# google/deepconsensus

Measured on NVIDIA H100. Metric: zmw_windows_per_sec, higher is better.
Workload: dtype bf16

## Files before the change

deepconsensus_b200/csrc/common.h:

```cpp
#pragma once
#include <cuda_bf16.h>
#include <stdint.h>

namespace dcb {

constexpr int kTileM = 128;
constexpr int kD = 280;
constexpr int kDP = 288;
constexpr int kHeads = 2;
constexpr int kDH = 140;
constexpr int kDHP = 144;
constexpr int kQKVN = 3 * kHeads * kDHP;
constexpr int kQKVGroup = 144;
constexpr int kNC = 144;
constexpr int kVocab = 5;
constexpr int kFFChunk = 128;

constexpr int kXChunks = kDP / 4;
__host__ __device__ inline size_t act_image_elems(int k) { return (size_t)kTileM * k; }
__host__ __device__ inline size_t x_image_elems() { return (size_t)kTileM * kDP; }

struct EmbedCol {
  int16_t src_row;
  int16_t width;
// ... 50 lines not shown
  float scale = 1.f;
};

struct RowEpi {
  float* x;
  __nv_bfloat16* xb;
  const float* bias;
  const float* pe;
  const float* pe_img;
  const float* ln_g;
  const float* ln_b;
  int has_xold;
  int L;
};

struct HeadParams {
  const float* x;
  const float* ln_g;
  const float* ln_b;
  const float* wfc;
  const float* bfc;
  const float* gw8;
  const float* ab;
  uint8_t* bases;
  uint8_t* quals;
  float* probs;
  float* logits;
  int M;
  int L, Lw;
  int calib_enabled;
// ... 7 lines not shown
```

deepconsensus_b200/csrc/engine.cu:

```cuda
#include <cuda_bf16.h>
#include <cuda_runtime.h>
#include <math.h>
#include <stdarg.h>
#include <stdio.h>
#include <string.h>

#include <algorithm>
#include <cmath>
#include <functional>
#include <map>
#include <memory>
#include <string>
#include <vector>

#include "../../include/dcb200.h"
#include "../../include/dcb200_debug.h"
#include "kernels.h"

using namespace dcb;

namespace {

thread_local std::string g_create_error;

// ... 97 lines not shown
  float prof_ms[kProfKinds] = {};
  int prof_n[kProfKinds] = {};
  long long prof_ffn_tokens = 0;
  float last_ms = 0.f;
  int last_launches = 0;
  int last_chunk_tokens = 0;
  std::vector<EmbedTable> tables;
  std::vector<StrictEmbedRow> embed;
  int table_elems = 0;
  Weights w;
  DevBuf<__nv_bfloat16> d_embqkv;
  DevBuf<float> d_x;
  DevBuf<__nv_bfloat16> d_xb;
  DevBuf<__nv_bfloat16> d_att;
  DevBuf<__nv_bfloat16> d_hid;
  DevBuf<double> d_p10;
  DevBuf<float> d_dbg;
  DevBuf<__nv_bfloat16> d_dbg_op;
  struct Strict {
    DevBuf<float> emb, x, y, q, k, v, att, hid;
    int chunk_windows = 0;
  } strict;
  struct {
    DevBuf<uint8_t> bases, quals, seq, qual, names, fastq;
    DevBuf<int32_t> start, len, pos, name_off, outcome;
    DevBuf<int64_t> rec_off, win_off;
    DevBuf<double> avg_q;
  } st;
  struct { DevBuf<int16_t> bq; DevBuf<uint8_t> mask; DevBuf<double> avg; } sk;
  struct {
// ... 477 lines not shown
    const int tl = t / e->L * e->Lw + t % e->L;
    const int tile = tl / kTileM, r = tl % kTileM;
    for (int col = 0; col < ow; ++col)
      out[(size_t)t * ow + col] = img[(((size_t)tile * (iw / K) + col / K) * kTileM + r) * K + col % K];
  }
  return DCB_OK;
}

void bf16_forward_chunk(dcb_engine* e, LaunchRecorder& rec, const float* rows_chunk, const uint8_t* packed_chunk,
                        int bw, HeadParams hp, int* d_status) {
  const dcb_config& c = e->cfg;
  const Weights& W = e->w;
  const int L = e->L, Lw = e->Lw, M = bw * Lw;
  const int T = (M + kTileM - 1) / kTileM;
  const cudaStream_t st = rec.st;
  int stage = 0;
  auto snap = [&]() {
    if (e->debug) {
      const size_t ximg = x_image_elems(), cw = (size_t)e->chunk_tiles * kTileM;
      cudaMemcpyAsync(e->d_dbg + (size_t)stage * e->chunk_tiles * ximg, e->d_x, T * ximg * sizeof(float), cudaMemcpyDeviceToDevice, st);
      size_t cols = 0;
      for (const DbgImage& im : dbg_images(e)) {
        if (im.stage == stage)
          cudaMemcpyAsync(e->d_dbg_op + cols * cw, im.src->p, (size_t)T * kTileM * im.width * sizeof(__nv_bfloat16),
                          cudaMemcpyDeviceToDevice, st);
        cols += im.width;
      }
    }
    ++stage;
  };
  rec.run(kProfEmbed, 1, [&] {
    launch_embed(rows_chunk, packed_chunk, e->pl, e->R, L, Lw, M, T, e->echunks, W.cols, W.rowmeta, W.tables,
                 e->table_elems, e->d_embqkv, d_status, st);
  });
  rec.run(kProfRowGemm, 1, [&] {
    launch_gemm_row(e->d_embqkv, W.wc, e->Epad / 16, 2 * (e->Epad / 16), T, row_epi(e, false, nullptr, 0, 0, true), st);
  });
  snap();
  for (int n_ = 0; n_ < c.num_hidden_layers; ++n_) {
    const LayerDev& ld = W.layers[n_];
    if (Lw == kTileM) {
      rec.run(kProfAttention, 2, [&] {
        __nv_bfloat16* qkv = e->debug ? e->d_embqkv.p : nullptr;
        for (int half = 0; half < 2; ++half)
          launch_qkv_attention(half, e->d_xb, ld.wqkv, L, c.attn_win_size, T, qkv, e->d_att, st);
      });
    } else {
      rec.run(kProfQkv, 1, [&] { launch_gemm_qkv(e->d_xb, ld.wqkv, T, e->d_embqkv, st); });
      rec.run(kProfAttention, 1, [&] { launch_attention(e->d_embqkv, e->d_att, L, Lw, c.attn_win_size, bw, st); });
    }
    rec.run(kProfRowGemm, 1, [&] {
      launch_gemm_row(e->d_att, ld.wo, kDP / 16, 2 * (kDP / 16), T, row_epi(e, true, nullptr, n_, 1, false), st);
    });
    snap();
    rec.run(kProfFfn, 2, [&] {
      const RowEpi epi = row_epi(e, true, ld.b2, n_ + 1, 0, false);
      __nv_bfloat16* hid = e->debug ? e->d_hid.p : nullptr;
      for (int half = 0; half < 2; ++half) launch_ffn(half, e->d_xb, ld.w1, ld.b1, ld.w2, c.filter_size, T, hid, epi, st);
    });
    if (e->profile) e->prof_ffn_tokens += (long long)bw * L;
    snap();
  }
  hp.x = e->d_x; hp.M = M; hp.L = L; hp.Lw = Lw;
  rec.run(kProfHead, 1, [&] { launch_head(hp, T, st); });
  e->last_chunk_tokens = M;
}

}

extern "C" {

const char* dcb_version(void) { return "dcb200 0.1.0 (sm_90a)"; }

const char* dcb_last_error(const dcb_engine* e) { return e ? e->err.c_str() : g_create_error.c_str(); }

int dcb_create(const dcb_config* cfg, dcb_engine** out) {
  if (!cfg || !out) return fail(nullptr, DCB_ERR_INVALID, "null argument");
  if (cfg->struct_size != (int32_t)sizeof(dcb_config))
    return fail(nullptr, DCB_ERR_INVALID, "dcb_config size mismatch: got %d, built with %zu",
// ... 13 lines not shown
  int ndev = 0;
  if (cudaGetDeviceCount(&ndev) != cudaSuccess || ndev == 0)
    return fail(nullptr, DCB_ERR_CUDA, "no CUDA device available (the dcb200 engine has no CPU fallback)");
  if (cfg->device < 0 || cfg->device >= ndev) return fail(nullptr, DCB_ERR_INVALID, "bad device ordinal %d", cfg->device);
  cudaDeviceProp prop;
  if (cudaGetDeviceProperties(&prop, cfg->device) != cudaSuccess || prop.major != 9)
    return fail(nullptr, DCB_ERR_CUDA, "device %d is not an sm_90 GPU (compute capability %d.%d)", cfg->device,
                prop.major, prop.minor);

  std::unique_ptr<dcb_engine> eng(new dcb_engine());
  dcb_engine* e = eng.get();
  e->cfg = *cfg;
  e->num_sms = prop.multiProcessorCount;
  e->L = cfg->max_length;
  e->Lw = e->L;
  bool align = true;
#ifdef DCB_DEV_SWITCHES
  if (const char* env = getenv("DCB_ALIGN")) align = atoi(env) != 0;
#endif
  if (align && e->L <= kTileM) e->Lw = kTileM;
  e->R = 4 * cfg->max_passes + (cfg->use_ccs_bq ? 6 : 5);
  e->pl = make_packed_layout(cfg->max_passes, cfg->max_length, cfg->use_ccs_bq ? 1 : 0);
  {
    auto table = [&](const char* layer, int vocab, int width) {
      const int off = (e->table_elems + 7) / 8 * 8;
      e->tables.push_back(EmbedTable{layer, vocab, width, off});
      e->table_elems = off + vocab * width;
      return e->tables.back();
    };
    auto rows = [&](const EmbedTable& tb, int n, float clip, int shift) {
      for (int r = 0; r < n; ++r) {
        e->embed.push_back(StrictEmbedRow{clip, shift, tb.vocab, tb.width, e->E, tb.off});
        e->E += tb.width;
      }
    };
// ... 32 lines not shown
    CU(e, kernels_init());
    std::vector<double> p10(256);
    for (int q = 0; q < 256; ++q) p10[q] = pow(10.0, (double)q / -10.0);
    int rc = upload(e, e->d_p10, p10);
    const size_t T = e->chunk_tiles, mtok = (size_t)cfg->max_batch * e->L;
    for (auto& sl : e->slots) {
      if (!rc) rc = alloc(e, sl.d_rows, (size_t)cfg->max_batch * e->R * e->L);
      if (!rc) rc = alloc(e, sl.d_status, 1);
      if (!rc) rc = alloc(e, sl.d_bases, mtok);
      if (!rc) rc = alloc(e, sl.d_quals, mtok);
    }
    if (!rc) rc = alloc(e, e->d_embqkv, T * kTileM * (size_t)std::max(e->Epad, kQKVN));
    if (!rc) rc = alloc(e, e->d_x, T * x_image_elems());
    if (!rc) rc = alloc(e, e->d_xb, T * act_image_elems(kDP));
    if (!rc) rc = alloc(e, e->d_att, T * act_image_elems(kDP));
    return rc;
  }();
  if (rc) {
    g_create_error = e->err;
    return rc;
  }
  *out = eng.release();
  return DCB_OK;
}

void dcb_destroy(dcb_engine* e) {
  if (!e) return;
  cudaSetDevice(e->cfg.device);
  delete e;
}
// ... 194 lines not shown
  if (!sl.used) { e->last_ms = 0.f; e->last_launches = 0; return DCB_OK; }
  CU(e, cudaSetDevice(e->cfg.device));
  CU(e, cudaEventSynchronize(sl.done));
  CU(e, cudaGetLastError());
  CU(e, cudaEventElapsedTime(&e->last_ms, sl.ev0, sl.ev1));
  e->last_launches = sl.launches;
  const int status = *sl.h_status;
  for (size_t i = 0; i < sl.prof_used; ++i) {
    const ProfRegion& r = sl.prof[i];
    float ms = 0.f;
    CU(e, cudaEventElapsedTime(&ms, r.start, r.end));
    e->prof_ms[r.kind] += ms;
    ++e->prof_n[r.kind];
  }
  sl.prof_used = 0;
  if (status & 1) return fail(e, DCB_ERR_INPUT_RANGE, "embedding id out of range in the input rows (clamped)");
  return DCB_OK;
}

int dcb_forward(dcb_engine* e, const float* rows, int32_t batch, uint32_t flags, uint8_t* bases_out,
                uint8_t* quals_out, float* probs_out, float* logits_out) {
  int64_t ticket = -1;
  int rc = dcb_submit(e, rows, batch, flags, bases_out, quals_out, probs_out, logits_out, &ticket);
  if (rc) return rc;
  return dcb_wait(e, ticket);
}

int dcb_last_forward_ms(dcb_engine* e, float* ms) {
  if (!e || !ms) return DCB_ERR_INVALID;
  *ms = e->last_ms;
// ... 727 lines not shown
```

deepconsensus_b200/csrc/kernels.cu:

```cuda
#include "kernels.h"

#include <cuda_bf16.h>
#include <math.h>
#include <stdio.h>
#include <stdlib.h>

#include "head_finish.cuh"
#include "sm90.cuh"

namespace dcb {


__global__ void __launch_bounds__(256)
embed_rows_kernel(const float* __restrict__ rows, const uint8_t* __restrict__ packed, PackedLayout pl, int R, int L,
                  int Lw, int M, int echunks,
                  const EmbedCol* __restrict__ cols, const EmbedRow* __restrict__ rowmeta,
                  const __nv_bfloat16* __restrict__ tables, int table_elems,
                  __nv_bfloat16* __restrict__ emb, int* __restrict__ status) {
  extern __shared__ __align__(1024) uint8_t smem[];
  __nv_bfloat16* s_tab = reinterpret_cast<__nv_bfloat16*>(smem);
  const int tab_bytes = (table_elems * 2 + 15) & ~15;
  EmbedCol* s_cols = reinterpret_cast<EmbedCol*>(smem + tab_bytes);
  const int cols_bytes = (echunks * 8 * (int)sizeof(EmbedCol) + 15) & ~15;
  uint16_t* s_ids = reinterpret_cast<uint16_t*>(smem + tab_bytes + cols_bytes);
  const int tile = blockIdx.x;
  for (int i = threadIdx.x; i < table_elems; i += blockDim.x) s_tab[i] = tables[i];
  for (int i = threadIdx.x; i < echunks * 8; i += blockDim.x) s_cols[i] = cols[i];
  for (int idx = threadIdx.x; idx < R * kTileM; idx += blockDim.x) {
    const int rr = idx / kTileM, r = idx % kTileM;
    const int tok = tile * kTileM + r;
    int id = 0;
    if (tok < M) {
      const int b = tok / Lw, l = tok - b * Lw;
      const EmbedRow m = rowmeta[rr];
// ... 29 lines not shown
          const EmbedCol c = s_cols[kc * 8 + 2 * j + h];
          uint32_t bits = 0;
          if (c.src_row >= 0) {
            const int id = s_ids[c.src_row * kTileM + r];
            bits = __bfloat16_as_ushort(s_tab[c.table_off + id * c.width + c.col]);
          }
          pr |= bits << (16 * h);
        }
        packed[j] = pr;
      }
      val = make_uint4(packed[0], packed[1], packed[2], packed[3]);
    }
    uint4* dst = reinterpret_cast<uint4*>(emb + ((size_t)tile * echunks + kc) * kTileM * 8) + r;
    *dst = val;
  }
}

enum { EPI_QKV = 0, EPI_ROW = 1 };

template <int BN, int NCH, bool kAres>
struct GemmCfg {
  static constexpr int kNI = NCH * BN;
  static constexpr int kSK = 2;
  static constexpr int kABytesPerK = 2 * kTileM * 16;
  static constexpr int kBBytesPerK = 2 * kNI * 16;
  static constexpr int kStageBytes = kSK * ((kAres ? 0 : kABytesPerK) + kBBytesPerK);
  static constexpr int kStages = 8;
  static constexpr int kShortStages = 4;
  static constexpr int kLongK = 32;
  __host__ __device__ static constexpr int stages(int kstages) {
// ... 107 lines not shown
          v1 = col + 1 < kD ? (v1 - mean) * rstd * s_vec[kDP + col + 1] + s_vec[2 * kDP + col + 1] : 0.f;
        }
        *reinterpret_cast<uint32_t*>(xb + (j * BN + jj * 8) * kTileM) = pack_bf16x2(v0, v1);
      }
  }
#pragma unroll
  for (int j = 0; j < NCH; ++j)
#pragma unroll
    for (int i = 0; i < BN / 2; ++i) acc[j][i] = 0.f;
}

template <int BN, int NCH, int EPI, bool kAres>
__global__ void __launch_bounds__(384, 1)
gemm_kernel(const __nv_bfloat16* __restrict__ a_img, const __nv_bfloat16* __restrict__ b_img, int a_ksteps, int ksteps,
            int ntiles,
            int ngroups, __nv_bfloat16* __restrict__ out_img, int out_chunks, RowEpi epi) {
  using Cfg = GemmCfg<BN, NCH, kAres>;
  static_assert(EPI != EPI_ROW || (Cfg::kNI == kDP && !kAres), "row epilogue needs the full 288-wide row");
  extern __shared__ __align__(1024) uint8_t smem[];
  uint8_t* a_res = smem;
  const int kstages = ksteps / Cfg::kSK;
  const int nst = Cfg::stages(kstages);
  uint8_t* stage_base = smem + Cfg::kAresBytes;
  uint64_t* full = reinterpret_cast<uint64_t*>(stage_base + nst * Cfg::kStageBytes);
  uint64_t* empty = full + nst;
  uint64_t* a_full = empty + nst;
  uint64_t* a_empty = a_full + 1;
  uint64_t* turn = a_empty + 1;
  float* s_vec = reinterpret_cast<float*>(stage_base + nst * Cfg::kStageBytes + 256);

  const int warp = threadIdx.x >> 5;
  const int lane = threadIdx.x & 31;
  if constexpr (EPI == EPI_ROW) row_vectors_to_smem(s_vec, epi);
  if (threadIdx.x == 0) {
    for (int i = 0; i < nst; ++i) {
      mbar_init(&full[i], 1);
      mbar_init(&empty[i], 256);
    }
    mbar_init(a_full, 1);
    mbar_init(a_empty, 256);
    mbar_init(&turn[0], 128);
    mbar_init(&turn[1], 128);
    mbar_fence_init();
  }
  __syncthreads();

  const int nitems = kAres ? (ntiles + 1) / 2 : ntiles * ngroups;
  const int gper = kAres ? ngroups : 1;
  const size_t a_tile_bytes = (size_t)a_ksteps * Cfg::kABytesPerK;
  const size_t b_group_bytes = (size_t)ksteps * Cfg::kBBytesPerK;

  if (warp >= 8) {
    setmaxnreg_dec<40>();
    if (warp == 8 && lane == 0) {
      uint32_t slot = 0, phase = 0, it = 0;
      for (int item = blockIdx.x; item < nitems; item += gridDim.x, ++it) {
        const int tile = kAres ? 2 * item : item / ngroups;
        const uint8_t* a_src = reinterpret_cast<const uint8_t*>(a_img) + tile * a_tile_bytes;
        if constexpr (kAres) {
          const uint32_t a_bytes = (uint32_t)((tile + 1 < ntiles ? 2 : 1) * a_tile_bytes);
          mbar_wait(a_empty, (it & 1) ^ 1);
          mbar_arrive_expect_tx(a_full, a_bytes);
          bulk_g2s(a_res, a_src, a_bytes, a_full);
        }
        for (int gi = 0; gi < gper; ++gi) {
          const int grp = kAres ? gi : item % ngroups;
          const uint8_t* b_src = reinterpret_cast<const uint8_t*>(b_img) + grp * b_group_bytes;
          for (int s = 0; s < kstages; ++s) {
            constexpr int kh = Cfg::kSK;
            mbar_wait(&empty[slot], phase ^ 1);
            uint8_t* st = stage_base + slot * Cfg::kStageBytes;
            if constexpr (kAres) {
              mbar_arrive_expect_tx(&full[slot], kh * Cfg::kBBytesPerK);
// ... 96 lines not shown
            const int row = row0 + 64 * mh + 8 * h;
#pragma unroll
            for (int j = 0; j < NCH; ++j)
#pragma unroll
              for (int jj = 0; jj < BN / 8; ++jj) {
                const int col = grp * Cfg::kNI + j * BN + jj * 8 + 2 * q;
                *reinterpret_cast<uint32_t*>(obase + ((size_t)(col >> 3) * kTileM + row) * 8 + (col & 7)) =
                    pack_bf16x2(accm[mh][j][jj * 4 + 2 * h], accm[mh][j][jj * 4 + 2 * h + 1]);
              }
          }
        if constexpr (kAres) pass_turn();
      } else {
        row_epilogue<BN, NCH>(accm[0], tile, row0, q, s_vec, epi);
      }
    }
  }
}

struct FfnCfg {
  static constexpr int kUpK = kDP / 16;
  static constexpr int kDownK = kFFChunk / 16;
  static constexpr int kABytesPerK = 2 * kTileM * 16;
  static constexpr int kW1Bytes = 2 * kFFChunk * 16;
  static constexpr int kW2Bytes = 2 * kDP * 16;
  static constexpr int kStageBytes = kW2Bytes;
  static constexpr int kB1Off = 2 * kW1Bytes;
  static constexpr int kB1Bytes = kFFChunk * 4;
  static constexpr int kStages = 16;
  static constexpr int kATileBytes = kUpK * kABytesPerK;
  static constexpr int kBarBytes = 512;
  static constexpr int kVecBytes = 3 * kDP * 4;
  static constexpr int kSmemBytes = kATileBytes + kStages * kStageBytes + kBarBytes + kVecBytes;
  static constexpr int kThreads = 384;
  static_assert(kSmemBytes <= 232448, "over the sm_90 opt-in shared memory per block");
  static_assert((2 * kStages + 2) * 8 <= kBarBytes, "the mbarriers (full, empty, a_full, a_empty) fit");
  static_assert(kB1Off + kB1Bytes <= kStageBytes && kUpK % 2 == 0, "a stage holds two W1 k-steps and b1");
};

template <bool kHid>
__global__ void __launch_bounds__(384, 1)
ffn_gemm_kernel(const __nv_bfloat16* __restrict__ xb_img, const __nv_bfloat16* __restrict__ w1_img,
                const float* __restrict__ b1, const __nv_bfloat16* __restrict__ w2_img, int ff, int tile_begin,
                int tile_end, __nv_bfloat16* __restrict__ hid, RowEpi epi) {
  using Cfg = FfnCfg;
  extern __shared__ __align__(1024) uint8_t smem[];
  uint8_t* a_res = smem;
  uint8_t* stage_base = smem + Cfg::kATileBytes;
  uint64_t* full = reinterpret_cast<uint64_t*>(stage_base + Cfg::kStages * Cfg::kStageBytes);
  uint64_t* empty = full + Cfg::kStages;
  uint64_t* a_full = empty + Cfg::kStages;
  uint64_t* a_empty = a_full + 1;
  float* s_vec = reinterpret_cast<float*>(reinterpret_cast<uint8_t*>(full) + Cfg::kBarBytes);
  const int nch = ff / kFFChunk;

  const int warp = threadIdx.x >> 5;
  const int lane = threadIdx.x & 31;
  row_vectors_to_smem(s_vec, epi);
  if (threadIdx.x == 0) {
    for (int i = 0; i < Cfg::kStages; ++i) {
      mbar_init(&full[i], 1);
      mbar_init(&empty[i], 256);
    }
    mbar_init(a_full, 1);
    mbar_init(a_empty, 256);
    mbar_fence_init();
  }
  __syncthreads();

  if (warp >= 8) {
    setmaxnreg_dec<24>();
    if (warp == 8 && lane == 0) {
      uint32_t slot = 0, phase = 0, it = 0;
      auto stage = [&](const uint8_t* src, uint32_t bytes, const float* b1_src, uint32_t b1_bytes) {
        mbar_wait(&empty[slot], phase ^ 1);
        uint8_t* st = stage_base + slot * Cfg::kStageBytes;
        mbar_arrive_expect_tx(&full[slot], bytes + b1_bytes);
        bulk_g2s(st, src, bytes, &full[slot]);
        if (b1_bytes) bulk_g2s(st + Cfg::kB1Off, b1_src, b1_bytes, &full[slot]);
        if (++slot == Cfg::kStages) { slot = 0; phase ^= 1; }
      };
      for (int tile = tile_begin + blockIdx.x; tile < tile_end; tile += gridDim.x, ++it) {
        mbar_wait(a_empty, (it & 1) ^ 1);
        mbar_arrive_expect_tx(a_full, Cfg::kATileBytes);
        bulk_g2s(a_res, reinterpret_cast<const uint8_t*>(xb_img) + (size_t)tile * Cfg::kATileBytes, Cfg::kATileBytes,
                 a_full);
        for (int c = 0; c < nch; ++c) {
          const uint8_t* w1 = reinterpret_cast<const uint8_t*>(w1_img) + (size_t)c * Cfg::kUpK * Cfg::kW1Bytes;
          for (int s = 0; s < Cfg::kUpK / 2; ++s)
            stage(w1 + (size_t)s * 2 * Cfg::kW1Bytes, 2 * Cfg::kW1Bytes, b1 + c * kFFChunk,
                  s + 1 == Cfg::kUpK / 2 ? Cfg::kB1Bytes : 0);
          const uint8_t* w2 = reinterpret_cast<const uint8_t*>(w2_img) + (size_t)c * Cfg::kDownK * Cfg::kW2Bytes;
          for (int kk = 0; kk < Cfg::kDownK; ++kk) stage(w2 + (size_t)kk * Cfg::kW2Bytes, Cfg::kW2Bytes, nullptr, 0);
        }
      }
    }
    return;
// ... 73 lines not shown
        if (kk > 0) {
          wgmma_fence_regs(af[kk - 1]);
          mbar_arrive(&empty[prev]);
        }
        prev = slot;
        next_slot();
      }
      wgmma_wait<0>();
      wgmma_fence_regs(acc[0]);
      wgmma_fence_regs(acc[1]);
      wgmma_fence_regs(af[Cfg::kDownK - 1]);
      mbar_arrive(&empty[prev]);
    }

    row_epilogue<kNC, 2, false>(acc, tile, row0, q, s_vec, epi);
  }
}

constexpr int kAttStride = 144;
constexpr int kAttChunks = kDHP / 8;

__device__ __forceinline__ void mma_bf16_16816(float (&c)[4], const uint32_t (&a)[4], uint32_t b0,
                                               uint32_t b1) {
  asm volatile(
      "mma.sync.aligned.m16n8k16.row.col.f32.bf16.bf16.f32 {%0,%1,%2,%3}, {%4,%5,%6,%7}, {%8,%9}, "
      "{%0,%1,%2,%3};"
      : "+f"(c[0]), "+f"(c[1]), "+f"(c[2]), "+f"(c[3])
      : "r"(a[0]), "r"(a[1]), "r"(a[2]), "r"(a[3]), "r"(b0), "r"(b1));
}

__device__ __forceinline__ void ldmatrix_x2_trans(uint32_t& r0, uint32_t& r1, uint32_t addr) {
// ... 218 lines not shown
  static constexpr int kKVBytes = kTileM * kAttStride * 2;
  static constexpr int kBarBytes = 256;
  static constexpr int kSmemBytes = kATileBytes + 2 * kKVBytes + kStages * kStageBytes + kBarBytes;
  static constexpr int kThreads = 384;
  static_assert(kSmemBytes <= 232448, "over the sm_90 opt-in shared memory per block");
  static_assert((2 * kStages + 2) * 8 <= kBarBytes, "the mbarriers (full, empty, a_full, a_empty) fit");
  static_assert((2 * kAK) % kSK == 0, "every stage holds kSK k-steps of one group");
  static_assert(kQKVGroup == kDHP && kQKVN == 6 * kQKVGroup, "one n-group is one head's q, k or v");
};

__device__ __forceinline__ int qkv_att_group(int i) {
  const int h = i / 3, part = i % 3;
  return part == 0 ? 2 + h : part == 1 ? 4 + h : h;
}

__device__ __forceinline__ void consumer_bar_sync() { asm volatile("bar.sync 1, 256;" ::: "memory"); }

template <bool kQkv>
__global__ void __launch_bounds__(384, 1)
qkv_attention_kernel(const __nv_bfloat16* __restrict__ xb_img, const __nv_bfloat16* __restrict__ b_img, int L,
                     int win, int tile_begin, int tile_end, __nv_bfloat16* __restrict__ qkv_img,
                     __nv_bfloat16* __restrict__ att) {
  using Cfg = QkvAttCfg;
  extern __shared__ __align__(1024) uint8_t smem[];
  uint8_t* a_res = smem;
  __nv_bfloat16* sK = reinterpret_cast<__nv_bfloat16*>(smem + Cfg::kATileBytes);
  __nv_bfloat16* sV = reinterpret_cast<__nv_bfloat16*>(smem + Cfg::kATileBytes + Cfg::kKVBytes);
  uint8_t* stage_base = smem + Cfg::kATileBytes + 2 * Cfg::kKVBytes;
  uint64_t* full = reinterpret_cast<uint64_t*>(stage_base + Cfg::kStages * Cfg::kStageBytes);
  uint64_t* empty = full + Cfg::kStages;
  uint64_t* a_full = empty + Cfg::kStages;
  uint64_t* a_empty = a_full + 1;

  const int warp = threadIdx.x >> 5;
  const int lane = threadIdx.x & 31;
  if (threadIdx.x == 0) {
    for (int i = 0; i < Cfg::kStages; ++i) {
      mbar_init(&full[i], 1);
      mbar_init(&empty[i], 256);
    }
    mbar_init(a_full, 1);
    mbar_init(a_empty, 256);
    mbar_fence_init();
  }
  __syncthreads();

  if (warp >= 8) {
    setmaxnreg_dec<24>();
    if (warp == 8 && lane == 0) {
      uint32_t slot = 0, phase = 0, it = 0;
      for (int tile = tile_begin + blockIdx.x; tile < tile_end; tile += gridDim.x, ++it) {
        mbar_wait(a_empty, (it & 1) ^ 1);
        mbar_arrive_expect_tx(a_full, Cfg::kATileBytes);
        bulk_g2s(a_res, reinterpret_cast<const uint8_t*>(xb_img) + (size_t)tile * Cfg::kATileBytes, Cfg::kATileBytes,
                 a_full);
        for (int i = 0; i < 6; ++i) {
          const uint8_t* b_src = reinterpret_cast<const uint8_t*>(b_img) + (size_t)qkv_att_group(i) * Cfg::kGroupBytes;
          for (int s = 0; s < Cfg::kGroupStages; ++s) {
            mbar_wait(&empty[slot], phase ^ 1);
            mbar_arrive_expect_tx(&full[slot], Cfg::kStageBytes);
            bulk_g2s(stage_base + slot * Cfg::kStageBytes, b_src + (size_t)s * Cfg::kStageBytes, Cfg::kStageBytes,
                     &full[slot]);
            if (++slot == Cfg::kStages) { slot = 0; phase ^= 1; }
          }
        }
      }
// ... 74 lines not shown
        } else {
          const bool v0 = row0 < L, v1 = row0 + 8 < L;
#pragma unroll
          for (int ks = 0; ks < kDHP / 16; ++ks) {
            qa[ks][0] = v0 ? pack_bf16x2(acc[8 * ks + 0], acc[8 * ks + 1]) : 0u;
            qa[ks][1] = v1 ? pack_bf16x2(acc[8 * ks + 2], acc[8 * ks + 3]) : 0u;
            qa[ks][2] = v0 ? pack_bf16x2(acc[8 * ks + 4], acc[8 * ks + 5]) : 0u;
            qa[ks][3] = v1 ? pack_bf16x2(acc[8 * ks + 6], acc[8 * ks + 7]) : 0u;
          }
        }
      }
      consumer_bar_sync();
      const int i0 = warp * 16;
      if (i0 < L) attend_block(qa, sK, sV, i0, L, band, att, tile * kTileM, h);
    }
  }
}

__global__ void __launch_bounds__(128)
head_kernel(HeadParams p) {
  __shared__ __align__(16) float sGW[kD * 8];
  __shared__ float sA[kVocab], sBj[kVocab];
  for (int i = threadIdx.x; i < kD * 2; i += blockDim.x)
    reinterpret_cast<float4*>(sGW)[i] = __ldg(reinterpret_cast<const float4*>(p.gw8) + i);
  if (threadIdx.x < kVocab) { sA[threadIdx.x] = p.ab[threadIdx.x]; sBj[threadIdx.x] = p.ab[8 + threadIdx.x]; }
  __syncthreads();
  const int tile = blockIdx.x, r = threadIdx.x;
  const int tok = tile * kTileM + r;
  if (tok >= p.M) return;
  const int wdw = tok / p.Lw, pos = tok - wdw * p.Lw;
  if (pos >= p.L) return;
  const size_t oidx = (size_t)wdw * p.L + pos;
  const float4* xrow = reinterpret_cast<const float4*>(p.x + (size_t)tile * x_image_elems()) + r;
  float s1 = 0.f, s2 = 0.f;
  float t[kVocab];
#pragma unroll
  for (int j = 0; j < kVocab; ++j) t[j] = 0.f;
  const float shift = xrow[0].x;
  constexpr int kHB = 10;
  static_assert((kD / 4) % kHB == 0, "head batch");
#pragma unroll 1
  for (int c0 = 0; c0 < kD / 4; c0 += kHB) {
// ... 9 lines not shown
        s1 += ys[i];
        s2 = fmaf(ys[i], ys[i], s2);
        const float4 w0 = *reinterpret_cast<const float4*>(&sGW[col * 8]);
        const float w4 = sGW[col * 8 + 4];
        t[0] = fmaf(ys[i], w0.x, t[0]); t[1] = fmaf(ys[i], w0.y, t[1]); t[2] = fmaf(ys[i], w0.z, t[2]);
        t[3] = fmaf(ys[i], w0.w, t[3]); t[4] = fmaf(ys[i], w4, t[4]);
      }
    }
  }
  const float m1 = s1 * (1.f / kD);
  const float rstd = rsqrtf(fmaxf(s2 * (1.f / kD) - m1 * m1, 0.f) + 1e-6f);
  float lg[kVocab];
#pragma unroll
  for (int j = 0; j < kVocab; ++j) lg[j] = rstd * (t[j] - m1 * sA[j]) + sBj[j];
  head_finish(p, lg, oidx);
}

static int g_num_sms = 0;
static int num_sms() {
  if (!g_num_sms) {
    int dev = 0;
    cudaGetDevice(&dev);
    cudaDeviceGetAttribute(&g_num_sms, cudaDevAttrMultiProcessorCount, dev);
    if (g_num_sms <= 0) g_num_sms = 132;
  }
  return g_num_sms;
}


template <int BN, int NCH, int EPI, bool kAres>
// ... 8 lines not shown
  if ((e = gemm_init<kNC, 1, EPI_QKV, true>()) != cudaSuccess) return e;
  for (auto fn : {ffn_gemm_kernel<false>, ffn_gemm_kernel<true>})
    if ((e = cudaFuncSetAttribute(fn, cudaFuncAttributeMaxDynamicSharedMemorySize, FfnCfg::kSmemBytes)) != cudaSuccess)
      return e;
  for (auto fn : {qkv_attention_kernel<false>, qkv_attention_kernel<true>})
    if ((e = cudaFuncSetAttribute(fn, cudaFuncAttributeMaxDynamicSharedMemorySize, QkvAttCfg::kSmemBytes)) !=
        cudaSuccess)
      return e;
  e = cudaFuncSetAttribute(embed_rows_kernel, cudaFuncAttributeMaxDynamicSharedMemorySize, 160 * 1024);
  if (e != cudaSuccess) return e;
  e = cudaFuncSetAttribute(band_attention_kernel, cudaFuncAttributeMaxDynamicSharedMemorySize,
                           2 * 256 * kAttStride * 2);
  return e;
}

size_t embed_smem_bytes(int R, int echunks, int table_elems) {
  return (size_t)((table_elems * 2 + 15) & ~15) + ((echunks * 8 * sizeof(EmbedCol) + 15) & ~(size_t)15) +
         (size_t)R * kTileM * 2;
}

void launch_embed(const float* rows, const uint8_t* packed, const PackedLayout& pl, int R, int L, int Lw, int M, int ntiles, int echunks,
                  const EmbedCol* cols, const EmbedRow* rowmeta, const __nv_bfloat16* tables,
                  int table_elems, __nv_bfloat16* emb, int* status, cudaStream_t st) {
  embed_rows_kernel<<<ntiles, 256, embed_smem_bytes(R, echunks, table_elems), st>>>(
      rows, packed, pl, R, L, Lw, M, echunks, cols, rowmeta, tables, table_elems, emb, status);
}

void launch_gemm_row(const __nv_bfloat16* a_img, const __nv_bfloat16* b_img, int a_ksteps, int b_ksteps, int ntiles,
                     const RowEpi& epi, cudaStream_t st) {
  using Cfg = GemmCfg<kNC, 2, false>;
  const int grid = ntiles < num_sms() ? ntiles : num_sms();
  const int smem = Cfg::smem_bytes(Cfg::stages(b_ksteps / Cfg::kSK));
  gemm_kernel<kNC, 2, EPI_ROW, false><<<grid, Cfg::kThreads, smem, st>>>(a_img, b_img, a_ksteps, b_ksteps, ntiles, 1,
                                                                                    nullptr, 0, epi);
}

void launch_gemm_qkv(const __nv_bfloat16* a_img, const __nv_bfloat16* b_img, int ntiles,
                     __nv_bfloat16* qkv_img, cudaStream_t st) {
  using Cfg = GemmCfg<kNC, 1, true>;
  const int npairs = (ntiles + 1) / 2;
  const int grid = npairs < num_sms() ? npairs : num_sms();
  RowEpi none{};
  gemm_kernel<kNC, 1, EPI_QKV, true><<<grid, Cfg::kThreads, Cfg::kSmemBytes, st>>>(
      a_img, b_img, kDP / 16, 2 * (kDP / 16), ntiles, kQKVN / kQKVGroup, qkv_img, kQKVN / 8, none);
}

void launch_ffn(int half, const __nv_bfloat16* xb_img, const __nv_bfloat16* w1_img, const float* b1,
                const __nv_bfloat16* w2_img, int ff, int ntiles, __nv_bfloat16* hid_img, const RowEpi& epi,
                cudaStream_t st) {
  const int split = (ntiles + 1) / 2;
  const int t0 = half ? split : 0, t1 = half ? ntiles : split;
  const int n = t1 - t0;
  const int grid = n < 1 ? 1 : n < num_sms() ? n : num_sms();
  if (hid_img)
    ffn_gemm_kernel<true><<<grid, FfnCfg::kThreads, FfnCfg::kSmemBytes, st>>>(xb_img, w1_img, b1, w2_img, ff, t0, t1,
                                                                              hid_img, epi);
  else
    ffn_gemm_kernel<false><<<grid, FfnCfg::kThreads, FfnCfg::kSmemBytes, st>>>(xb_img, w1_img, b1, w2_img, ff, t0, t1,
                                                                               nullptr, epi);
}

__global__ void __launch_bounds__(256)
unpack_rows_kernel(const uint8_t* __restrict__ packed, PackedLayout pl, int nwindows, float* __restrict__ rows) {
  const int b = blockIdx.x;
  const uint8_t* w = packed + (size_t)b * pl.stride;
  float* out = rows + (size_t)b * pl.R * pl.L;
  for (int i = threadIdx.x; i < pl.R * pl.L; i += blockDim.x) {
    const int r = i / pl.L, l = i - r * pl.L;
    out[i] = packed_value(pl, w, r, l);
  }
}

void launch_unpack_rows(const uint8_t* packed, const PackedLayout& pl, int nwindows, float* rows, cudaStream_t st) {
  if (nwindows > 0) unpack_rows_kernel<<<nwindows, 256, 0, st>>>(packed, pl, nwindows, rows);
}


void launch_attention(const __nv_bfloat16* qkv, __nv_bfloat16* att, int L, int Lw, int win, int nwindows,
                      cudaStream_t st) {
  const int Lp = (L + 15) & ~15;
  const size_t smem = (size_t)2 * Lp * kAttStride * 2;
  band_attention_kernel<<<nwindows * 2, 128, smem, st>>>(qkv, att, L, Lw, win, nwindows);
}

void launch_qkv_attention(int half, const __nv_bfloat16* xb_img, const __nv_bfloat16* wqkv, int L, int win,
                          int ntiles, __nv_bfloat16* qkv_img, __nv_bfloat16* att, cudaStream_t st) {
  const int split = (ntiles + 1) / 2;
  const int t0 = half ? split : 0, t1 = half ? ntiles : split;
  const int n = t1 - t0;
  const int grid = n < 1 ? 1 : n < num_sms() ? n : num_sms();
  if (qkv_img)
    qkv_attention_kernel<true><<<grid, QkvAttCfg::kThreads, QkvAttCfg::kSmemBytes, st>>>(xb_img, wqkv, L, win, t0, t1,
                                                                                        qkv_img, att);
  else
    qkv_attention_kernel<false><<<grid, QkvAttCfg::kThreads, QkvAttCfg::kSmemBytes, st>>>(xb_img, wqkv, L, win, t0,
                                                                                         t1, nullptr, att);
}



__global__ void __launch_bounds__(256)
stitch_kernel(const uint8_t* __restrict__ bases, const uint8_t* __restrict__ quals, int L,
              const int64_t* __restrict__ win_off, const int32_t* __restrict__ zmw_start, uint8_t* __restrict__ seq_out,
              uint8_t* __restrict__ qual_out, int32_t* __restrict__ len_out) {
  __shared__ int s_warp[8];
  __shared__ int s_total;
  const int z = blockIdx.x;
  const size_t off = (size_t)window_offset(win_off, zmw_start[z], L);
  const int n = (int)(window_offset(win_off, zmw_start[z + 1], L) - (int64_t)off);
  const uint8_t* in_b = bases + off;
  const uint8_t* in_q = quals + off;
// ... 33 lines not shown
        out_q[pos] = q[k];
        ++pos;
      }
    }
    running += s_total;
    __syncthreads();
  }
  if (threadIdx.x == 0) len_out[z] = running;
}

void launch_stitch(const uint8_t* bases, const uint8_t* quals, int L, const int64_t* win_off, const int32_t* zmw_start,
                   int n_zmw, uint8_t* seq_out, uint8_t* qual_out, int32_t* len_out, cudaStream_t st) {
  if (n_zmw > 0) stitch_kernel<<<n_zmw, 256, 0, st>>>(bases, quals, L, win_off, zmw_start, seq_out, qual_out, len_out);
}

void launch_head(const HeadParams& p, int ntiles, cudaStream_t st) {
  head_kernel<<<ntiles, 128, 0, st>>>(p);
}

}
```

deepconsensus_b200/csrc/kernels.h:

```cpp
#pragma once
#include <cuda_runtime.h>

#include "common.h"

namespace dcb {

cudaError_t kernels_init();

size_t embed_smem_bytes(int R, int echunks, int table_elems);
void launch_embed(const float* rows, const uint8_t* packed, const PackedLayout& pl, int R, int L, int Lw, int M, int ntiles, int echunks,
                  const EmbedCol* cols, const EmbedRow* rowmeta, const __nv_bfloat16* tables,
                  int table_elems, __nv_bfloat16* emb, int* status, cudaStream_t st);
void launch_gemm_row(const __nv_bfloat16* a_img, const __nv_bfloat16* b_img, int a_ksteps, int b_ksteps, int ntiles,
                     const RowEpi& epi, cudaStream_t st);
void launch_gemm_qkv(const __nv_bfloat16* a_img, const __nv_bfloat16* b_img, int ntiles,
                     __nv_bfloat16* qkv_img, cudaStream_t st);
void launch_ffn(int half, const __nv_bfloat16* xb_img, const __nv_bfloat16* w1_img, const float* b1,
                const __nv_bfloat16* w2_img, int ff, int ntiles, __nv_bfloat16* hid_img, const RowEpi& epi,
                cudaStream_t st);
void launch_unpack_rows(const uint8_t* packed, const PackedLayout& pl, int nwindows, float* rows, cudaStream_t st);
void launch_attention(const __nv_bfloat16* qkv, __nv_bfloat16* att, int L, int Lw, int win, int nwindows,
                      cudaStream_t st);
void launch_qkv_attention(int half, const __nv_bfloat16* xb_img, const __nv_bfloat16* wqkv, int L, int win,
                          int ntiles, __nv_bfloat16* qkv_img, __nv_bfloat16* att, cudaStream_t st);
void launch_head(const HeadParams& p, int ntiles, cudaStream_t st);
__host__ __device__ inline int64_t window_offset(const int64_t* win_off, int w, int L) {
  return win_off ? win_off[w] : (int64_t)w * L;
}
void launch_stitch(const uint8_t* bases, const uint8_t* quals, int L, const int64_t* win_off, const int32_t* zmw_start,
                   int n_zmw, uint8_t* seq_out, uint8_t* qual_out, int32_t* len_out, cudaStream_t st);


void launch_read_outcome(const uint8_t* qual, const int32_t* len, const int64_t* win_off, const int32_t* zmw_start,
                         const int32_t* window_pos, int L, int n_zmw, const double* p10, double min_quality, int min_length,
                         int32_t* outcome, double* avg_q, cudaStream_t st);
void launch_fastq(const uint8_t* seq, const uint8_t* qual, const int32_t* len, const int64_t* win_off, const int32_t* zmw_start,
                  int L, int n_zmw, const int32_t* outcome, const uint8_t* names, const int32_t* name_off, int64_t* rec_off,
                  uint8_t* fastq, int64_t cap, cudaStream_t st);
void launch_skip_mask(const int16_t* ccs_bq, int n_windows, int L, const double* p10, double thr, uint8_t* mask,
                      double* avg_out, cudaStream_t st);
// ... 72 lines not shown
```

Before: 165,000.

## Overlap forward kernels with PDL and per-tile release/acquire flags

Kernels in the forward pass are launched with programmatic stream serialization, so each can start while the one before is still running. Per-tile stamp flags in global memory, written with release stores and polled with acquire loads, let a consumer tile begin as soon as the matching producer tile is done, instead of waiting at a full kernel boundary. This targets launch gaps and tail idle time between the many kernels per layer. It adds spin-wait polling with a one-second timeout that reports an error, plus stamp bookkeeping, and it risks deadlock or extra contention if CTAs of the dependent kernel take SM slots the producer still needs.

```diff
diff --git a/deepconsensus_b200/csrc/common.h b/deepconsensus_b200/csrc/common.h
--- a/deepconsensus_b200/csrc/common.h
+++ b/deepconsensus_b200/csrc/common.h
@@ -88,6 +88,13 @@
   int L;
 };
 
+struct TileFlow {
+  int* flags;
+  int wait, done;
+  int* status;
+};
+constexpr int kStatusTileWait = 2;
+
 struct HeadParams {
   const float* x;
   const float* ln_g;
diff --git a/deepconsensus_b200/csrc/engine.cu b/deepconsensus_b200/csrc/engine.cu
--- a/deepconsensus_b200/csrc/engine.cu
+++ b/deepconsensus_b200/csrc/engine.cu
@@ -135,6 +135,9 @@
   DevBuf<__nv_bfloat16> d_xb;
   DevBuf<__nv_bfloat16> d_att;
   DevBuf<__nv_bfloat16> d_hid;
+  DevBuf<int> d_flow;
+  uint32_t flow_stamp = 0;
+  bool tile_flow = false;
   DevBuf<double> d_p10;
   DevBuf<float> d_dbg;
   DevBuf<__nv_bfloat16> d_dbg_op;
@@ -642,6 +645,23 @@
   const int L = e->L, Lw = e->Lw, M = bw * Lw;
   const int T = (M + kTileM - 1) / kTileM;
   const cudaStream_t st = rec.st;
+  const bool flow = e->tile_flow;
+  const uint32_t nstamps = 3 + 3 * (uint32_t)c.num_hidden_layers;
+  if (flow && e->flow_stamp > UINT32_MAX - nstamps) {
+    cudaMemsetAsync(e->d_flow, 0, e->chunk_tiles * sizeof(int), st);
+    e->flow_stamp = 0;
+  }
+  auto next_flow = [&](bool advance = true) {
+    TileFlow f{};
+    if (flow) {
+      f.flags = e->d_flow;
+      f.status = d_status;
+      f.wait = (int)e->flow_stamp;
+      f.done = (int)(e->flow_stamp + 1);
+      if (advance) ++e->flow_stamp;
+    }
+    return f;
+  };
   int stage = 0;
   auto snap = [&]() {
     if (e->debug) {
@@ -659,10 +679,11 @@
   };
   rec.run(kProfEmbed, 1, [&] {
     launch_embed(rows_chunk, packed_chunk, e->pl, e->R, L, Lw, M, T, e->echunks, W.cols, W.rowmeta, W.tables,
-                 e->table_elems, e->d_embqkv, d_status, st);
+                 e->table_elems, e->d_embqkv, d_status, next_flow(), st);
   });
   rec.run(kProfRowGemm, 1, [&] {
-    launch_gemm_row(e->d_embqkv, W.wc, e->Epad / 16, 2 * (e->Epad / 16), T, row_epi(e, false, nullptr, 0, 0, true), st);
+    launch_gemm_row(e->d_embqkv, W.wc, e->Epad / 16, 2 * (e->Epad / 16), T, row_epi(e, false, nullptr, 0, 0, true),
+                    next_flow(), st);
   });
   snap();
   for (int n_ = 0; n_ < c.num_hidden_layers; ++n_) {
@@ -671,26 +692,28 @@
       rec.run(kProfAttention, 2, [&] {
         __nv_bfloat16* qkv = e->debug ? e->d_embqkv.p : nullptr;
         for (int half = 0; half < 2; ++half)
-          launch_qkv_attention(half, e->d_xb, ld.wqkv, L, c.attn_win_size, T, qkv, e->d_att, st);
+          launch_qkv_attention(half, e->d_xb, ld.wqkv, L, c.attn_win_size, T, qkv, e->d_att, next_flow(half == 1), st);
       });
     } else {
       rec.run(kProfQkv, 1, [&] { launch_gemm_qkv(e->d_xb, ld.wqkv, T, e->d_embqkv, st); });
       rec.run(kProfAttention, 1, [&] { launch_attention(e->d_embqkv, e->d_att, L, Lw, c.attn_win_size, bw, st); });
     }
     rec.run(kProfRowGemm, 1, [&] {
-      launch_gemm_row(e->d_att, ld.wo, kDP / 16, 2 * (kDP / 16), T, row_epi(e, true, nullptr, n_, 1, false), st);
+      launch_gemm_row(e->d_att, ld.wo, kDP / 16, 2 * (kDP / 16), T, row_epi(e, true, nullptr, n_, 1, false), next_flow(),
+                      st);
     });
     snap();
     rec.run(kProfFfn, 2, [&] {
       const RowEpi epi = row_epi(e, true, ld.b2, n_ + 1, 0, false);
       __nv_bfloat16* hid = e->debug ? e->d_hid.p : nullptr;
-      for (int half = 0; half < 2; ++half) launch_ffn(half, e->d_xb, ld.w1, ld.b1, ld.w2, c.filter_size, T, hid, epi, st);
+      for (int half = 0; half < 2; ++half)
+        launch_ffn(half, e->d_xb, ld.w1, ld.b1, ld.w2, c.filter_size, T, hid, epi, next_flow(half == 1), st);
     });
     if (e->profile) e->prof_ffn_tokens += (long long)bw * L;
     snap();
   }
   hp.x = e->d_x; hp.M = M; hp.L = L; hp.Lw = Lw;
-  rec.run(kProfHead, 1, [&] { launch_head(hp, T, st); });
+  rec.run(kProfHead, 1, [&] { launch_head(hp, T, next_flow(), st); });
   e->last_chunk_tokens = M;
 }
 
@@ -734,11 +757,13 @@
   e->num_sms = prop.multiProcessorCount;
   e->L = cfg->max_length;
   e->Lw = e->L;
-  bool align = true;
+  bool align = true, tile_flow = true;
 #ifdef DCB_DEV_SWITCHES
   if (const char* env = getenv("DCB_ALIGN")) align = atoi(env) != 0;
+  if (const char* env = getenv("DCB_TILE_FLOW")) tile_flow = atoi(env) != 0;
 #endif
   if (align && e->L <= kTileM) e->Lw = kTileM;
+  e->tile_flow = tile_flow && e->Lw == kTileM;
   e->R = 4 * cfg->max_passes + (cfg->use_ccs_bq ? 6 : 5);
   e->pl = make_packed_layout(cfg->max_passes, cfg->max_length, cfg->use_ccs_bq ? 1 : 0);
   {
@@ -801,6 +826,7 @@
     if (!rc) rc = alloc(e, e->d_x, T * x_image_elems());
     if (!rc) rc = alloc(e, e->d_xb, T * act_image_elems(kDP));
     if (!rc) rc = alloc(e, e->d_att, T * act_image_elems(kDP));
+    if (!rc && e->tile_flow) rc = alloc(e, e->d_flow, T);
     return rc;
   }();
   if (rc) {
@@ -1025,6 +1051,9 @@
     ++e->prof_n[r.kind];
   }
   sl.prof_used = 0;
+  if (status & kStatusTileWait)
+    return fail(e, DCB_ERR_CUDA, "a launch of the forward waited over a second for a tile of the launch before it; "
+                                 "the outputs are not valid");
   if (status & 1) return fail(e, DCB_ERR_INPUT_RANGE, "embedding id out of range in the input rows (clamped)");
   return DCB_OK;
 }
diff --git a/deepconsensus_b200/csrc/kernels.cu b/deepconsensus_b200/csrc/kernels.cu
--- a/deepconsensus_b200/csrc/kernels.cu
+++ b/deepconsensus_b200/csrc/kernels.cu
@@ -10,14 +10,43 @@
 
 namespace dcb {
 
+__device__ __forceinline__ void pdl_launch_dependents() { asm volatile("griddepcontrol.launch_dependents;" ::: "memory"); }
+__device__ __forceinline__ void pdl_wait() { asm volatile("griddepcontrol.wait;" ::: "memory"); }
+
+__device__ __forceinline__ int ld_acquire_gpu(const int* p) {
+  int v;
+  asm volatile("ld.acquire.gpu.global.b32 %0, [%1];" : "=r"(v) : "l"(p) : "memory");
+  return v;
+}
+
+__device__ __forceinline__ void tile_wait(const TileFlow& f, int tile) {
+  if (!f.flags) return;
+  if (ld_acquire_gpu(f.flags + tile) == f.wait) return;
+  uint64_t t0, t;
+  asm volatile("mov.u64 %0, %%globaltimer;" : "=l"(t0));
+  while (ld_acquire_gpu(f.flags + tile) != f.wait) {
+    __nanosleep(100);
+    asm volatile("mov.u64 %0, %%globaltimer;" : "=l"(t));
+    if (t - t0 > 1000000000ull) { atomicOr(f.status, kStatusTileWait); return; }
+  }
+}
+
+__device__ __forceinline__ void fence_proxy_async() { asm volatile("fence.proxy.async.global;" ::: "memory"); }
+
+__device__ __forceinline__ void tile_done(const TileFlow& f, int tile) {
+  if (f.flags) asm volatile("st.release.gpu.global.b32 [%0], %1;" ::"l"(f.flags + tile), "r"(f.done) : "memory");
+}
+
+__device__ __forceinline__ void consumer_bar_sync() { asm volatile("bar.sync 1, 256;" ::: "memory"); }
 
 __global__ void __launch_bounds__(256)
 embed_rows_kernel(const float* __restrict__ rows, const uint8_t* __restrict__ packed, PackedLayout pl, int R, int L,
                   int Lw, int M, int echunks,
                   const EmbedCol* __restrict__ cols, const EmbedRow* __restrict__ rowmeta,
                   const __nv_bfloat16* __restrict__ tables, int table_elems,
-                  __nv_bfloat16* __restrict__ emb, int* __restrict__ status) {
+                  __nv_bfloat16* __restrict__ emb, int* __restrict__ status, TileFlow flow) {
   extern __shared__ __align__(1024) uint8_t smem[];
+  pdl_launch_dependents();
   __nv_bfloat16* s_tab = reinterpret_cast<__nv_bfloat16*>(smem);
   const int tab_bytes = (table_elems * 2 + 15) & ~15;
   EmbedCol* s_cols = reinterpret_cast<EmbedCol*>(smem + tab_bytes);
@@ -77,6 +106,8 @@
     uint4* dst = reinterpret_cast<uint4*>(emb + ((size_t)tile * echunks + kc) * kTileM * 8) + r;
     *dst = val;
   }
+  __syncthreads();
+  if (threadIdx.x == 0) tile_done(flow, tile);
 }
 
 enum { EPI_QKV = 0, EPI_ROW = 1 };
@@ -214,7 +245,7 @@
 __global__ void __launch_bounds__(384, 1)
 gemm_kernel(const __nv_bfloat16* __restrict__ a_img, const __nv_bfloat16* __restrict__ b_img, int a_ksteps, int ksteps,
             int ntiles,
-            int ngroups, __nv_bfloat16* __restrict__ out_img, int out_chunks, RowEpi epi) {
+            int ngroups, __nv_bfloat16* __restrict__ out_img, int out_chunks, RowEpi epi, TileFlow flow) {
   using Cfg = GemmCfg<BN, NCH, kAres>;
   static_assert(EPI != EPI_ROW || (Cfg::kNI == kDP && !kAres), "row epilogue needs the full 288-wide row");
   extern __shared__ __align__(1024) uint8_t smem[];
@@ -244,6 +275,7 @@
     mbar_fence_init();
   }
   __syncthreads();
+  pdl_launch_dependents();
 
   const int nitems = kAres ? (ntiles + 1) / 2 : ntiles * ngroups;
   const int gper = kAres ? ngroups : 1;
@@ -257,6 +289,8 @@
       for (int item = blockIdx.x; item < nitems; item += gridDim.x, ++it) {
         const int tile = kAres ? 2 * item : item / ngroups;
         const uint8_t* a_src = reinterpret_cast<const uint8_t*>(a_img) + tile * a_tile_bytes;
+        tile_wait(flow, tile);
+        fence_proxy_async();
         if constexpr (kAres) {
           const uint32_t a_bytes = (uint32_t)((tile + 1 < ntiles ? 2 : 1) * a_tile_bytes);
           mbar_wait(a_empty, (it & 1) ^ 1);
@@ -383,7 +417,12 @@
         row_epilogue<BN, NCH>(accm[0], tile, row0, q, s_vec, epi);
       }
     }
-  }
+    if (flow.flags) {
+      consumer_bar_sync();
+      if (threadIdx.x == 0) tile_done(flow, item);
+    }
+  }
+  pdl_wait();
 }
 
 struct FfnCfg {
@@ -410,7 +449,7 @@
 __global__ void __launch_bounds__(384, 1)
 ffn_gemm_kernel(const __nv_bfloat16* __restrict__ xb_img, const __nv_bfloat16* __restrict__ w1_img,
                 const float* __restrict__ b1, const __nv_bfloat16* __restrict__ w2_img, int ff, int tile_begin,
-                int tile_end, __nv_bfloat16* __restrict__ hid, RowEpi epi) {
+                int tile_end, __nv_bfloat16* __restrict__ hid, RowEpi epi, TileFlow flow) {
   using Cfg = FfnCfg;
   extern __shared__ __align__(1024) uint8_t smem[];
   uint8_t* a_res = smem;
@@ -435,6 +474,7 @@
     mbar_fence_init();
   }
   __syncthreads();
+  pdl_launch_dependents();
 
   if (warp >= 8) {
     setmaxnreg_dec<24>();
@@ -449,6 +489,8 @@
         if (++slot == Cfg::kStages) { slot = 0; phase ^= 1; }
       };
       for (int tile = tile_begin + blockIdx.x; tile < tile_end; tile += gridDim.x, ++it) {
+        tile_wait(flow, tile);
+        fence_proxy_async();
         mbar_wait(a_empty, (it & 1) ^ 1);
         mbar_arrive_expect_tx(a_full, Cfg::kATileBytes);
         bulk_g2s(a_res, reinterpret_cast<const uint8_t*>(xb_img) + (size_t)tile * Cfg::kATileBytes, Cfg::kATileBytes,
@@ -552,7 +594,12 @@
     }
 
     row_epilogue<kNC, 2, false>(acc, tile, row0, q, s_vec, epi);
-  }
+    if (flow.flags) {
+      consumer_bar_sync();
+      if (threadIdx.x == 0) tile_done(flow, tile);
+    }
+  }
+  pdl_wait();
 }
 
 constexpr int kAttStride = 144;
@@ -801,13 +848,11 @@
   return part == 0 ? 2 + h : part == 1 ? 4 + h : h;
 }
 
-__device__ __forceinline__ void consumer_bar_sync() { asm volatile("bar.sync 1, 256;" ::: "memory"); }
-
 template <bool kQkv>
 __global__ void __launch_bounds__(384, 1)
 qkv_attention_kernel(const __nv_bfloat16* __restrict__ xb_img, const __nv_bfloat16* __restrict__ b_img, int L,
                      int win, int tile_begin, int tile_end, __nv_bfloat16* __restrict__ qkv_img,
-                     __nv_bfloat16* __restrict__ att) {
+                     __nv_bfloat16* __restrict__ att, TileFlow flow) {
   using Cfg = QkvAttCfg;
   extern __shared__ __align__(1024) uint8_t smem[];
   uint8_t* a_res = smem;
@@ -831,12 +876,15 @@
     mbar_fence_init();
   }
   __syncthreads();
+  pdl_launch_dependents();
 
   if (warp >= 8) {
     setmaxnreg_dec<24>();
     if (warp == 8 && lane == 0) {
       uint32_t slot = 0, phase = 0, it = 0;
       for (int tile = tile_begin + blockIdx.x; tile < tile_end; tile += gridDim.x, ++it) {
+        tile_wait(flow, tile);
+        fence_proxy_async();
         mbar_wait(a_empty, (it & 1) ^ 1);
         mbar_arrive_expect_tx(a_full, Cfg::kATileBytes);
         bulk_g2s(a_res, reinterpret_cast<const uint8_t*>(xb_img) + (size_t)tile * Cfg::kATileBytes, Cfg::kATileBytes,
@@ -941,18 +989,16 @@
       const int i0 = warp * 16;
       if (i0 < L) attend_block(qa, sK, sV, i0, L, band, att, tile * kTileM, h);
     }
-  }
-}
-
-__global__ void __launch_bounds__(128)
-head_kernel(HeadParams p) {
-  __shared__ __align__(16) float sGW[kD * 8];
-  __shared__ float sA[kVocab], sBj[kVocab];
-  for (int i = threadIdx.x; i < kD * 2; i += blockDim.x)
-    reinterpret_cast<float4*>(sGW)[i] = __ldg(reinterpret_cast<const float4*>(p.gw8) + i);
-  if (threadIdx.x < kVocab) { sA[threadIdx.x] = p.ab[threadIdx.x]; sBj[threadIdx.x] = p.ab[8 + threadIdx.x]; }
-  __syncthreads();
-  const int tile = blockIdx.x, r = threadIdx.x;
+    if (flow.flags) {
+      consumer_bar_sync();
+      if (threadIdx.x == 0) tile_done(flow, tile);
+    }
+  }
+  pdl_wait();
+}
+
+__device__ __forceinline__ void head_row(const HeadParams& p, const float* sGW, const float* sA, const float* sBj,
+                                         int tile, int r) {
   const int tok = tile * kTileM + r;
   if (tok >= p.M) return;
   const int wdw = tok / p.Lw, pos = tok - wdw * p.Lw;
@@ -992,6 +1038,19 @@
 #pragma unroll
   for (int j = 0; j < kVocab; ++j) lg[j] = rstd * (t[j] - m1 * sA[j]) + sBj[j];
   head_finish(p, lg, oidx);
+}
+
+__global__ void __launch_bounds__(128)
+head_kernel(HeadParams p, TileFlow flow) {
+  __shared__ __align__(16) float sGW[kD * 8];
+  __shared__ float sA[kVocab], sBj[kVocab];
+  for (int i = threadIdx.x; i < kD * 2; i += blockDim.x)
+    reinterpret_cast<float4*>(sGW)[i] = __ldg(reinterpret_cast<const float4*>(p.gw8) + i);
+  if (threadIdx.x < kVocab) { sA[threadIdx.x] = p.ab[threadIdx.x]; sBj[threadIdx.x] = p.ab[8 + threadIdx.x]; }
+  if (threadIdx.x == 0) tile_wait(flow, blockIdx.x);
+  __syncthreads();
+  head_row(p, sGW, sA, sBj, blockIdx.x, threadIdx.x);
+  pdl_wait();
 }
 
 static int g_num_sms = 0;
@@ -1030,6 +1089,22 @@
   return e;
 }
 
+template <typename... P, typename... A>
+static void launch(const TileFlow& flow, void (*kernel)(P...), int grid, int threads, size_t smem, cudaStream_t st,
+                   A... args) {
+  cudaLaunchAttribute attr{};
+  attr.id = cudaLaunchAttributeProgrammaticStreamSerialization;
+  attr.val.programmaticStreamSerializationAllowed = 1;
+  cudaLaunchConfig_t cfg{};
+  cfg.gridDim = dim3(grid);
+  cfg.blockDim = dim3(threads);
+  cfg.dynamicSmemBytes = smem;
+  cfg.stream = st;
+  cfg.attrs = flow.flags ? &attr : nullptr;
+  cfg.numAttrs = flow.flags ? 1 : 0;
+  cudaLaunchKernelEx(&cfg, kernel, args...);
+}
+
 size_t embed_smem_bytes(int R, int echunks, int table_elems) {
   return (size_t)((table_elems * 2 + 15) & ~15) + ((echunks * 8 * sizeof(EmbedCol) + 15) & ~(size_t)15) +
          (size_t)R * kTileM * 2;
@@ -1037,18 +1112,18 @@
 
 void launch_embed(const float* rows, const uint8_t* packed, const PackedLayout& pl, int R, int L, int Lw, int M, int ntiles, int echunks,
                   const EmbedCol* cols, const EmbedRow* rowmeta, const __nv_bfloat16* tables,
-                  int table_elems, __nv_bfloat16* emb, int* status, cudaStream_t st) {
+                  int table_elems, __nv_bfloat16* emb, int* status, const TileFlow& flow, cudaStream_t st) {
   embed_rows_kernel<<<ntiles, 256, embed_smem_bytes(R, echunks, table_elems), st>>>(
-      rows, packed, pl, R, L, Lw, M, echunks, cols, rowmeta, tables, table_elems, emb, status);
+      rows, packed, pl, R, L, Lw, M, echunks, cols, rowmeta, tables, table_elems, emb, status, flow);
 }
 
 void launch_gemm_row(const __nv_bfloat16* a_img, const __nv_bfloat16* b_img, int a_ksteps, int b_ksteps, int ntiles,
-                     const RowEpi& epi, cudaStream_t st) {
+                     const RowEpi& epi, const TileFlow& flow, cudaStream_t st) {
   using Cfg = GemmCfg<kNC, 2, false>;
   const int grid = ntiles < num_sms() ? ntiles : num_sms();
   const int smem = Cfg::smem_bytes(Cfg::stages(b_ksteps / Cfg::kSK));
-  gemm_kernel<kNC, 2, EPI_ROW, false><<<grid, Cfg::kThreads, smem, st>>>(a_img, b_img, a_ksteps, b_ksteps, ntiles, 1,
-                                                                                    nullptr, 0, epi);
+  launch(flow, gemm_kernel<kNC, 2, EPI_ROW, false>, grid, Cfg::kThreads, smem, st, a_img, b_img, a_ksteps, b_ksteps,
+         ntiles, 1, (__nv_bfloat16*)nullptr, 0, epi, flow);
 }
 
 void launch_gemm_qkv(const __nv_bfloat16* a_img, const __nv_bfloat16* b_img, int ntiles,
@@ -1058,22 +1133,18 @@
   const int grid = npairs < num_sms() ? npairs : num_sms();
   RowEpi none{};
   gemm_kernel<kNC, 1, EPI_QKV, true><<<grid, Cfg::kThreads, Cfg::kSmemBytes, st>>>(
-      a_img, b_img, kDP / 16, 2 * (kDP / 16), ntiles, kQKVN / kQKVGroup, qkv_img, kQKVN / 8, none);
+      a_img, b_img, kDP / 16, 2 * (kDP / 16), ntiles, kQKVN / kQKVGroup, qkv_img, kQKVN / 8, none, TileFlow{});
 }
 
 void launch_ffn(int half, const __nv_bfloat16* xb_img, const __nv_bfloat16* w1_img, const float* b1,
                 const __nv_bfloat16* w2_img, int ff, int ntiles, __nv_bfloat16* hid_img, const RowEpi& epi,
-                cudaStream_t st) {
+                const TileFlow& flow, cudaStream_t st) {
   const int split = (ntiles + 1) / 2;
   const int t0 = half ? split : 0, t1 = half ? ntiles : split;
   const int n = t1 - t0;
   const int grid = n < 1 ? 1 : n < num_sms() ? n : num_sms();
-  if (hid_img)
-    ffn_gemm_kernel<true><<<grid, FfnCfg::kThreads, FfnCfg::kSmemBytes, st>>>(xb_img, w1_img, b1, w2_img, ff, t0, t1,
-                                                                              hid_img, epi);
-  else
-    ffn_gemm_kernel<false><<<grid, FfnCfg::kThreads, FfnCfg::kSmemBytes, st>>>(xb_img, w1_img, b1, w2_img, ff, t0, t1,
-                                                                               nullptr, epi);
+  launch(flow, hid_img ? ffn_gemm_kernel<true> : ffn_gemm_kernel<false>, grid, FfnCfg::kThreads, FfnCfg::kSmemBytes,
+         st, xb_img, w1_img, b1, w2_img, ff, t0, t1, hid_img, epi, flow);
 }
 
 __global__ void __launch_bounds__(256)
@@ -1100,17 +1171,14 @@
 }
 
 void launch_qkv_attention(int half, const __nv_bfloat16* xb_img, const __nv_bfloat16* wqkv, int L, int win,
-                          int ntiles, __nv_bfloat16* qkv_img, __nv_bfloat16* att, cudaStream_t st) {
+                          int ntiles, __nv_bfloat16* qkv_img, __nv_bfloat16* att, const TileFlow& flow,
+                          cudaStream_t st) {
   const int split = (ntiles + 1) / 2;
   const int t0 = half ? split : 0, t1 = half ? ntiles : split;
   const int n = t1 - t0;
   const int grid = n < 1 ? 1 : n < num_sms() ? n : num_sms();
-  if (qkv_img)
-    qkv_attention_kernel<true><<<grid, QkvAttCfg::kThreads, QkvAttCfg::kSmemBytes, st>>>(xb_img, wqkv, L, win, t0, t1,
-                                                                                        qkv_img, att);
-  else
-    qkv_attention_kernel<false><<<grid, QkvAttCfg::kThreads, QkvAttCfg::kSmemBytes, st>>>(xb_img, wqkv, L, win, t0,
-                                                                                         t1, nullptr, att);
+  launch(flow, qkv_img ? qkv_attention_kernel<true> : qkv_attention_kernel<false>, grid, QkvAttCfg::kThreads,
+         QkvAttCfg::kSmemBytes, st, xb_img, wqkv, L, win, t0, t1, qkv_img, att, flow);
 }
 
 
@@ -1174,8 +1242,8 @@
   if (n_zmw > 0) stitch_kernel<<<n_zmw, 256, 0, st>>>(bases, quals, L, win_off, zmw_start, seq_out, qual_out, len_out);
 }
 
-void launch_head(const HeadParams& p, int ntiles, cudaStream_t st) {
-  head_kernel<<<ntiles, 128, 0, st>>>(p);
-}
-
-}
+void launch_head(const HeadParams& p, int ntiles, const TileFlow& flow, cudaStream_t st) {
+  launch(flow, head_kernel, ntiles, 128, 0, st, p, flow);
+}
+
+}
diff --git a/deepconsensus_b200/csrc/kernels.h b/deepconsensus_b200/csrc/kernels.h
--- a/deepconsensus_b200/csrc/kernels.h
+++ b/deepconsensus_b200/csrc/kernels.h
@@ -10,20 +10,21 @@
 size_t embed_smem_bytes(int R, int echunks, int table_elems);
 void launch_embed(const float* rows, const uint8_t* packed, const PackedLayout& pl, int R, int L, int Lw, int M, int ntiles, int echunks,
                   const EmbedCol* cols, const EmbedRow* rowmeta, const __nv_bfloat16* tables,
-                  int table_elems, __nv_bfloat16* emb, int* status, cudaStream_t st);
+                  int table_elems, __nv_bfloat16* emb, int* status, const TileFlow& flow, cudaStream_t st);
 void launch_gemm_row(const __nv_bfloat16* a_img, const __nv_bfloat16* b_img, int a_ksteps, int b_ksteps, int ntiles,
-                     const RowEpi& epi, cudaStream_t st);
+                     const RowEpi& epi, const TileFlow& flow, cudaStream_t st);
 void launch_gemm_qkv(const __nv_bfloat16* a_img, const __nv_bfloat16* b_img, int ntiles,
                      __nv_bfloat16* qkv_img, cudaStream_t st);
 void launch_ffn(int half, const __nv_bfloat16* xb_img, const __nv_bfloat16* w1_img, const float* b1,
                 const __nv_bfloat16* w2_img, int ff, int ntiles, __nv_bfloat16* hid_img, const RowEpi& epi,
-                cudaStream_t st);
+                const TileFlow& flow, cudaStream_t st);
 void launch_unpack_rows(const uint8_t* packed, const PackedLayout& pl, int nwindows, float* rows, cudaStream_t st);
 void launch_attention(const __nv_bfloat16* qkv, __nv_bfloat16* att, int L, int Lw, int win, int nwindows,
                       cudaStream_t st);
 void launch_qkv_attention(int half, const __nv_bfloat16* xb_img, const __nv_bfloat16* wqkv, int L, int win,
-                          int ntiles, __nv_bfloat16* qkv_img, __nv_bfloat16* att, cudaStream_t st);
-void launch_head(const HeadParams& p, int ntiles, cudaStream_t st);
+                          int ntiles, __nv_bfloat16* qkv_img, __nv_bfloat16* att, const TileFlow& flow,
+                          cudaStream_t st);
+void launch_head(const HeadParams& p, int ntiles, const TileFlow& flow, cudaStream_t st);
 __host__ __device__ inline int64_t window_offset(const int64_t* win_off, int w, int L) {
   return win_off ? win_off[w] : (int64_t)w * L;
 }
```

After: 177,800 (median of 6 runs). 1.08x the previous value.
